# tumaer/lagrangebench

Measured on AMD Instinct MI355X. Metric: rollout particle-steps/sec, higher is better.
Workload: dtype f32 (GEMMs as fp16 hi/lo split products, fp32 accumulate)

## Files before the change

### include/lbhip.h

```cpp
#ifndef LBHIP_H
#define LBHIP_H

#include <stdint.h>

#ifdef __cplusplus
extern "C" {
#endif

#define LB_OK 0
#define LB_ERR_ARG (-1)
#define LB_ERR_HIP (-2)
#define LB_ERR_STATE (-3)
#define LB_ERR_DENSITY (-4)
#define LB_ERR_UNSUPPORTED (-5)

#define LB_FORCE_NONE 0
#define LB_FORCE_PIECEWISE 1
#define LB_FORCE_BUFFER 2

typedef struct lb_engine lb_engine;
typedef struct lb_gns lb_gns;

typedef struct lb_case_desc {
  int32_t dim;
// ... 38 lines not shown

int lb_set_force(lb_engine* eng, const double* force_dev);

int lb_load_window(lb_engine* eng, const double* traj_dev, int32_t T, int32_t t0, int32_t step);

int lb_read_window(lb_engine* eng, double* win_out_dev);


int lb_nl_allocate(lb_engine* eng, int32_t* cell_capacity_out, int32_t* e_cap_out,
                   int32_t* occupancy_out );

int lb_nl_set_capacity(lb_engine* eng, int32_t cell_capacity, int32_t e_cap);

int lb_nl_update(lb_engine* eng);

int lb_nl_read_flags(lb_engine* eng, int32_t* overflow_out_dev);

int lb_nl_read_idx(lb_engine* eng, int32_t* idx_out_dev, int32_t* n_edges_out_dev);


int lb_node_features(lb_engine* eng, double* vel_hist_out_dev, double* vel_mag_out_dev,
                     double* bound_out_dev, double* force_out_dev);

int lb_edge_features(lb_engine* eng, double* rel_disp_out_dev, double* rel_dist_out_dev);


int lb_gns_create(lb_engine* eng, const lb_gns_desc* desc, const float* weights_host,
                  int64_t n_floats, lb_gns** out);
void lb_gns_destroy(lb_gns* gns);

// ... 148 lines not shown
```

### lagrangebench_amd/_lib.py

```python
from __future__ import annotations

import ctypes as C
import os
from typing import Optional

_HERE = os.path.dirname(os.path.abspath(__file__))
LIB_PATH = os.path.join(_HERE, "csrc", "liblbhip.so")

LB_OK = 0
LB_FORCE_NONE, LB_FORCE_PIECEWISE, LB_FORCE_BUFFER = 0, 1, 2

D3 = C.c_double * 3


class CaseDesc(C.Structure):

    _fields_ = [
        ("dim", C.c_int32), ("n_particles", C.c_int32), ("batch", C.c_int32), ("isl", C.c_int32),
        ("periodic", C.c_int32), ("has_bound", C.c_int32), ("has_vel_mag", C.c_int32),
        ("force_kind", C.c_int32), ("force_axis", C.c_int32), ("geometry_f32", C.c_int32),
        ("box", D3), ("r_cutoff", C.c_double), ("capacity_multiplier", C.c_double),
        ("vel_mean", D3), ("vel_std", D3), ("acc_mean", D3), ("acc_std", D3),
        ("bound_lo", D3), ("bound_hi", D3),
        ("force_split", C.c_double), ("force_lo", D3), ("force_hi", D3),
# ... 45 lines not shown
_P = C.c_void_p
_SIGS = {
    "lb_strerror": (C.c_char_p, [C.c_int]),
    "lb_last_error": (C.c_char_p, []),
    "lb_version": (C.c_int, []),
    "lb_engine_create": (C.c_int, [C.POINTER(CaseDesc), _P, C.POINTER(_P)]),
    "lb_engine_destroy": (None, [_P]),
    "lb_set_particle_type": (C.c_int, [_P, _P]),
    "lb_set_force": (C.c_int, [_P, _P]),
    "lb_load_window": (C.c_int, [_P, _P, C.c_int32, C.c_int32, C.c_int32]),
    "lb_read_window": (C.c_int, [_P, _P]),
    "lb_nl_allocate": (C.c_int, [_P, C.POINTER(C.c_int32), C.POINTER(C.c_int32), C.POINTER(C.c_int32)]),
    "lb_nl_set_capacity": (C.c_int, [_P, C.c_int32, C.c_int32]),
    "lb_nl_update": (C.c_int, [_P]),
    "lb_nl_read_flags": (C.c_int, [_P, _P]),
    "lb_nl_read_idx": (C.c_int, [_P, _P, _P]),
    "lb_node_features": (C.c_int, [_P, _P, _P, _P, _P]),
    "lb_edge_features": (C.c_int, [_P, _P, _P]),
    "lb_gns_create": (C.c_int, [_P, C.POINTER(GnsDesc), _P, C.c_int64, C.POINTER(_P)]),
    "lb_gns_destroy": (None, [_P]),
    "lb_gns_forward": (C.c_int, [_P, _P, _P]),
    "lb_set_fused_aggregation": (C.c_int, [_P, C.c_int32]),
    "lb_gns_set_tap": (C.c_int, [_P, _P]),
    "lb_math_mode": (C.c_int, [_P, C.c_int32, C.POINTER(C.c_int32), C.POINTER(C.c_int32)]),
    "lb_math_fallbacks": (C.c_int32, [_P]),
    "lb_debug_inject_guard": (C.c_int, [_P, C.c_int32, C.c_int32]),
    "lb_integrate": (C.c_int, [_P, _P, _P, _P, C.c_int32]),
    "lb_case_integrate": (C.c_int, [_P, C.c_int32, _P, _P, C.c_int32, _P]),
    "lb_rollout": (C.c_int, [_P, _P, _P, C.c_int32, C.c_int32, _P, C.POINTER(C.c_int32)]),
    "lb_ekin": (C.c_int, [_P, _P, C.c_int32, C.c_int32, C.c_double, C.c_double, _P, C.c_int32]),
# ... 82 lines not shown
```

### lagrangebench_amd/csrc/lb_api.hip

```cpp
#include <cstddef>
#include <stdarg.h>
#include <stdio.h>
#include <stdlib.h>
#include <string.h>

#include <algorithm>
#include <cmath>

#include <initializer_list>
#include <tuple>

#include "lb_internal.h"
#include "lb_msplit.h"

thread_local std::string g_lb_err;

int lb_fail(int code, const char* fmt, ...) {
  char buf[1024];
  va_list ap;
  va_start(ap, fmt);
  vsnprintf(buf, sizeof(buf), fmt, ap);
  va_end(ap);
  g_lb_err = buf;
  return code;
// ... 221 lines not shown
  if (hipMemcpy(e->ctrl, &c0, sizeof(c0), hipMemcpyHostToDevice) != hipSuccess ||
      hipMemset(e->blocks_done, 0, sizeof(int32_t)) != hipSuccess ||
      hipMemset(e->ptype, 0, sizeof(int32_t) * BN) != hipSuccess ||
      hipMemset(e->nl_wg_sum, 0, sizeof(unsigned long long) * (BN / 8 + 2)) != hipSuccess ||
      hipMemset(e->row_ptr, 0, sizeof(int32_t) * (BN + 1)) != hipSuccess) {
    lb_engine_destroy(e);
    return lb_fail(LB_ERR_HIP, "engine init copies failed");
  }
  *out = e;
  return LB_OK;
}

extern "C" void lb_engine_destroy(lb_engine* e) {
  if (!e) return;
  lb_timers_collect(e);
  for (auto ev : e->epool) (void)hipEventDestroy(ev);
  void* bufs[] = {e->win, e->ptype, e->force, e->ctrl, e->cell_of, e->cell_count, e->cell_start,
                  e->cell_part, e->deg, e->nl_wg_sum, e->row_ptr, e->scan_part, e->cpos, e->tmp_send, e->tmp_feat, e->tmp_feat64,
                  e->senders, e->receivers, e->efeat, e->efeat64,
                  e->overflow, e->nedges_b, e->xnode, e->nlat, e->agg, e->psr, e->elat, e->msg,
                  e->acc, e->blocks_done};
  for (void* b : bufs)
    if (b) (void)hipFree(b);
  if (e->ctrl_host) (void)hipHostFree(e->ctrl_host);
  if (e->host_flag) (void)hipHostFree(e->host_flag);
  for (int i = 0; i < 4; ++i)
    if (e->step_ev[i]) (void)hipEventDestroy(e->step_ev[i]);
  if (e->gstream) (void)hipStreamDestroy(e->gstream);
  delete e;
}
// ... 114 lines not shown
    want = std::min<int32_t>(want, e->nl_dense ? LB_MAX_ROW_DENSE : LB_MAX_ROW);
    if (e->nl_dense) e->row_cap = std::max(e->row_cap, std::min<int32_t>((want + 63) / 64 * 64, LB_MAX_ROW_DENSE));
    if (want > e->maxd || !e->tmp_send) {
      LB_HIP(hipStreamSynchronize(e->stream));
      for (void* b : {(void*)e->tmp_send, (void*)e->tmp_feat, (void*)e->tmp_feat64})
        if (b) (void)hipFree(b);
      e->tmp_send = nullptr;
      e->tmp_feat = nullptr;
      e->tmp_feat64 = nullptr;
      e->maxd = want;
      LB_TRY(lb_alloc(&e->tmp_send, (size_t)e->BN * want));
      LB_TRY(lb_alloc(&e->tmp_feat, (size_t)e->BN * want * 4));
      LB_TRY(lb_alloc(&e->tmp_feat64, (size_t)e->BN * want * 4));
    }
  }
  if (cell_capacity_out) *cell_capacity_out = e->cell_capacity;
  if (e_cap_out) *e_cap_out = e->e_cap;
  if (occupancy_out) memcpy(occupancy_out, occ.data(), sizeof(int32_t) * e->g.B);
  return LB_OK;
}

extern "C" int lb_nl_set_capacity(lb_engine* e, int32_t cell_capacity, int32_t e_cap) {
  if (!e || e_cap < 1) return lb_fail(LB_ERR_ARG, "bad capacity");
  e->cell_capacity = cell_capacity;
  e->e_cap = e_cap;
  return lb_ensure_edges(e, (int64_t)e_cap * e->g.B);
}

extern "C" int lb_nl_update(lb_engine* e) {
  if (!e) return lb_fail(LB_ERR_ARG, "null engine");
// ... 672 lines not shown
      e->stream = s;
    }
  } restore{e, user_stream, &exec};
  if (use_graph) {
    if (!e->gstream) LB_HIP(hipStreamCreateWithFlags(&e->gstream, hipStreamNonBlocking));
    LB_HIP(hipEventRecord(e->step_ev[0], user_stream));
    LB_HIP(hipStreamWaitEvent(e->gstream, e->step_ev[0], 0));
    e->stream = e->gstream;
  }
  int n_realloc = 0, n_retry = 0;
  if (start_step > 0)
    LB_TRY(lbk_load_window_resume(e, traj_dev, T, pred_out_dev, n_steps, start_step));
  else
    LB_TRY(lbk_load_window(e, traj_dev, T, 0, 0));
  if (e->e_cap <= 0) LB_TRY(lb_nl_allocate(e, nullptr, nullptr, nullptr));
  int step = start_step;
  const int RA = 3;
  const int last = (stop_step >= 0 && stop_step < n_steps) ? stop_step : n_steps;
  while (step < last) {
    bool warm = false;
    for (int s = step; s < last; ++s) {
      if (s - step >= RA) {
        LB_HIP(hipEventSynchronize(e->step_ev[(s - RA) & 3]));
        if (*(volatile int32_t*)e->host_flag >= 0) break;
      }
      if (use_graph && warm && !exec) {
        hipGraph_t graph = nullptr;
        LB_HIP(hipStreamBeginCapture(e->stream, hipStreamCaptureModeThreadLocal));
        const int rc = lb_enqueue_step(e, forward, model, traj_dev, T, pred_out_dev, n_steps);
        const hipError_t ce = hipStreamEndCapture(e->stream, &graph);
// ... 36 lines not shown
      step = s_bad;
      if (++n_retry > 4) return lb_fail(LB_ERR_STATE, "single-launch paths keep timing out");
      continue;
    }
    LB_TRY(lb_check_density(e));
    if (e->ctrl_host->overflow_step < 0) break;
    step = e->ctrl_host->step;
    ++n_realloc;
    if (n_realloc > n_steps + 8) return lb_fail(LB_ERR_STATE, "neighbor list keeps overflowing");
    if (exec) {
      (void)hipGraphExecDestroy(exec);
      exec = nullptr;
    }
    LB_TRY(lb_nl_allocate(e, nullptr, nullptr, nullptr));
  }
  if (n_realloc_out) *n_realloc_out = n_realloc;
  return LB_OK;
}

extern "C" int lb_ekin(lb_engine* e, const double* rollout_dev, int32_t T, int32_t stride, double dt,
                       double dx, double* out_dev, int32_t n_out) {
  if (!e || !rollout_dev || !out_dev) return lb_fail(LB_ERR_ARG, "null argument");
  if (stride < 1 || T < 2) return lb_fail(LB_ERR_ARG, "need stride >= 1 and T >= 2");
  const int expect = (T - 1 + stride - 1) / stride;
  if (n_out != expect) return lb_fail(LB_ERR_ARG, "n_out must be ceil((T-1)/stride) = %d", expect);
  return lbk_ekin(e, rollout_dev, T, stride, n_out, dt, dx, out_dev);
}

extern "C" int lb_sinkhorn(lb_engine* e, const double* pred_dev, int32_t pred_T, const double* target_dev,
                           int32_t target_T, int32_t stride, double threshold, double* out_dev, int32_t n_out,
// ... 31 lines not shown
```

### lagrangebench_amd/csrc/lb_internal.h

```cpp
#pragma once
#include <cstdlib>
#include <hip/hip_ext.h>
#include <hip/hip_runtime.h>
#include <stdint.h>

#include <string>
#include <vector>

#include "../../include/lbhip.h"

#define LB_MAX_STENCIL_CAND 2048
#define LB_MAX_ROW 256
#define LB_MAX_ROW_DENSE 4096
#define LB_TILE 32
#define LB_D 128

typedef float f32x4 __attribute__((ext_vector_type(4)));
typedef float f32x16 __attribute__((ext_vector_type(16)));

struct lb_ctrl {
  int32_t step;
  int32_t overflow_step;
  int32_t n_edges_total;
  int32_t n_edges_unclamped;
  int32_t max_cell_occ;
  int32_t density_error;
  int32_t max_deg;
  int32_t row_overflow;
  int32_t math_flags;
  float ln_inv_d;
  float ln_pad;
  int32_t persist_error;
  int32_t nl_epoch;
  int32_t persist_step;
  int32_t math_step;
  int32_t acct_builds;
  int32_t acct_first;
  int64_t acct_sum;
};
__device__ __forceinline__ void lb_acct_edges(lb_ctrl* ctrl, int total) {
  if (ctrl->acct_builds == 0) ctrl->acct_first = total;
  ctrl->acct_builds += 1;
  ctrl->acct_sum += total;
}
#define LB_MATH_NO_STEP 0x7fffffff
#define LB_MATH_LARGE 1
#define LB_MATH_TINY 2
#define LB_MATH_NONFINITE 4

struct lb_geom {
  int32_t dim, N, B, isl, periodic, has_bound, has_vel_mag, force_kind, force_axis;
  int32_t use_cell_list;
  int32_t ncell[3];
// ... 71 lines not shown
  int32_t cell_capacity, e_cap;
  int64_t e_alloc;
  int32_t* cell_of;
  int32_t* cell_count;
  int32_t* cell_start;
  int32_t* cell_fill;
  bool cells_traj_ready = false;
  int32_t* cell_part;
  int32_t* deg;
  lb_feat_job feat_job{};
  bool feat_done = false;
  lb_integ_job integ_job{};
  bool integ_done = false;
  bool nl_one_off = false;
  unsigned long long* nl_wg_sum = nullptr;
  int32_t* row_ptr;
  int32_t* scan_part;
  double* cpos;
  int64_t cell_slots = 0;
  bool nl_dense = false;
  int32_t row_cap = 0;
  int32_t maxd;
  int32_t* tmp_send;
  float* tmp_feat;
  double* tmp_feat64;
  int32_t* senders;
  int32_t* receivers;
  float* efeat;
  double* efeat64;
  int32_t* overflow;
// ... 161 lines not shown
#define LB_LAUNCH_TIMED(e, kern, grid, block, ...)                                                        \
  do {                                                                                                    \
    if ((e)->ext_armed && !(e)->ext_used) {                                                               \
      hipExtLaunchKernelGGL(kern, grid, block, 0, (e)->stream, (e)->trecs.back().a, (e)->trecs.back().b, \
                            0, __VA_ARGS__);                                                              \
      (e)->ext_used = true;                                                                               \
    } else {                                                                                              \
      hipLaunchKernelGGL(kern, grid, block, 0, (e)->stream, __VA_ARGS__);                                 \
    }                                                                                                     \
  } while (0)

int lb_ensure_edges(lb_engine* e, int64_t need);
int lb_alloc_aggpart(lb_engine* e);

int lbk_nl_build(lb_engine* e, bool want_efeat64);
int lbk_nl_export(lb_engine* e, int32_t* idx_out, int32_t* n_edges_out);
int lbk_edge_features_export(lb_engine* e, double* rel_disp, double* rel_dist);

int lbk_load_window(lb_engine* e, const double* traj, int T, int t0, int step);
int lbk_load_window_resume(lb_engine* e, const double* traj, int T, const double* pred, int pred_T, int step);
int lbk_read_window(lb_engine* e, double* out);
int lbk_node_features(lb_engine* e, float* xnode, const float* embed, int emb, int ntypes,
                      double* vel_hist, double* vel_mag, double* bound, double* force);
int lbk_integrate(lb_engine* e, const float* acc, int acc_stride, const double* target,
                  const double* traj, int T, double* pred, int pred_T);
int lbk_ekin(lb_engine* e, const double* roll, int T, int stride, int n_out, double dt, double dx,
             double* out);
int lbk_case_integrate(lb_engine* e, int mode, const float* pred, const double* pos_seq, int T,
                       double* out);
int lbk_metrics(lb_engine* e, const double* pred, int pred_T, const double* target, int target_T,
// ... 74 lines not shown
```

### lagrangebench_amd/csrc/lb_neighbor.hip

```cpp
#include "lb_features.h"

#define SCAN_THREADS 256
#define SCAN_CHUNK (SCAN_THREADS * 8)
#define NL_SMALL_MAXC 1024

enum { NL_COUNT = 0, NL_FILL = 1, NL_ROWS = 2 };

__global__ void k_cell_count(lb_geom g, int64_t BN, const double* __restrict__ win,
                             lb_ctrl* __restrict__ ctrl, int32_t* __restrict__ cell_of,
                             int32_t* __restrict__ cell_count) {
  if (ctrl->overflow_step >= 0) return;
  int64_t gi = (int64_t)blockIdx.x * blockDim.x + threadIdx.x;
  if (gi == 0) {
    ctrl->max_cell_occ = 0;
    ctrl->max_deg = 0;
    ctrl->row_overflow = 0;
  }
  if (gi >= BN) return;
  const int step = ctrl->step;
  const int b = (int)(gi / g.N);
  int h = 0, mult = 1;
  for (int d = 0; d < g.dim; ++d) {
    double p = lb_pos(win, g, BN, step, g.isl - 1, d, gi);
    int c = __double2int_rz(lb_r(p / g.cell_size[d], g.f32));
// ... 85 lines not shown
  if (gi >= BN) return;
  const int step = ctrl->step;
  const int gc = cell_of[gi];
  const int slot = cell_start[gc] + atomicAdd(&cell_fill[gc], 1);
  cell_part[slot] = (int32_t)gi;
  for (int d = 0; d < g.dim; ++d) cpos[(int64_t)d * BN + slot] = lb_pos(win, g, BN, step, g.isl - 1, d, gi);
}

__global__ void k_cell_zero(lb_ctrl* __restrict__ ctrl, int32_t* __restrict__ cell_count, int n) {
  if (ctrl->overflow_step >= 0) return;
  const int i = blockIdx.x * blockDim.x + threadIdx.x;
  if (i == 0) {
    ctrl->max_cell_occ = 0;
    ctrl->max_deg = 0;
    ctrl->row_overflow = 0;
  }
  if (i < n) cell_count[i] = 0;
}
__global__ void __launch_bounds__(256) k_cell_bin(lb_geom g, int64_t BN, const double* __restrict__ win,
                                                  lb_ctrl* __restrict__ ctrl, int32_t* __restrict__ cell_of,
                                                  int32_t* __restrict__ cell_count, int32_t* __restrict__ cell_part,
                                                  double* __restrict__ cpos, int32_t cap, int64_t cstride) {
  if (ctrl->overflow_step >= 0) return;
  const int64_t gi = (int64_t)blockIdx.x * blockDim.x + threadIdx.x;
  const int step = ctrl->step;
  int occ = 0;
  if (gi < BN) {
    const int b = (int)(gi / g.N);
    int h = 0, mult = 1;
    double p[3] = {0, 0, 0};
// ... 269 lines not shown
  const int32_t* cell_start;
  const int32_t* cell_part;
  const double* cpos;
  const int32_t* cell_cnt;
  int32_t cell_cap;
  int64_t cstride;
  int32_t* deg;
  const int32_t* row_ptr;
  lb_edge_out out;
  int64_t e_alloc;
  int32_t maxd;
  int32_t row_cap;
  lb_feat_job feat;
  const double* win;
  int32_t nb_search;
};
#define NL_FEAT_ROWS 8
__device__ __forceinline__ int lb_cell_begin(const lb_nl_args& a, int gc) { return a.cell_cap ? gc * a.cell_cap : a.cell_start[gc]; }
__device__ __forceinline__ int lb_cell_size(const lb_nl_args& a, int gc, int begin) {
  return a.cell_cap ? min(a.cell_cnt[gc], a.cell_cap) : a.cell_start[gc + 1] - begin;
}


__device__ __forceinline__ void lb_load_pos(double* p, const double* src, int64_t stride, int64_t i, int dim) {
#pragma unroll
  for (int d = 0; d < 3; ++d) p[d] = d < dim ? src[d * stride + i] : 0.0;
}

template <bool F32, typename PS>
__device__ __forceinline__ bool lb_pair_in_cutoff(const lb_geom& g, PS ps, const double* pr, int dim) {
  double dd = lb_disp1(ps(0), pr[0], g.box[0], g.half_box[0], g.periodic, F32);
// ... 80 lines not shown
  return s_cstart[lo] + (j - s_coff[lo]);
}

__device__ __forceinline__ bool lb_feature_rows(const lb_geom& g, int64_t BN, const lb_ctrl* ctrl, const lb_nl_args& a,
                                                int waves) {
  if (a.nb_search <= 0 || (int)blockIdx.x < a.nb_search) return false;
  const int64_t first = ((int64_t)(blockIdx.x - a.nb_search) * waves + (threadIdx.x >> 6)) * NL_FEAT_ROWS;
  const int cnt = (int)min((int64_t)NL_FEAT_ROWS, BN - first);
  if (cnt > 0)
    lb_node_features_wave_multi(g, BN, a.win, ctrl->step, a.feat, [&](int p) -> int64_t { return first + p; }, cnt);
  return true;
}

template <int MODE>
__device__ __forceinline__ int lb_cap_row(lb_ctrl* ctrl, const lb_nl_args& a, int count, int lane, int row_cap, bool can_grow) {
  if (count > row_cap) {
    if (lane == 0) {
      if (MODE == NL_ROWS && can_grow)
        atomicExch(&ctrl->row_overflow, 1);
      else
        atomicExch(&ctrl->density_error, 2);
    }
    count = row_cap;
  }
  if (MODE == NL_ROWS && count > a.maxd) {
    if (lane == 0) atomicExch(&ctrl->row_overflow, 1);
    count = a.maxd;
  }
  return count;
}

__device__ __forceinline__ int lb_rank_in_row(int my, int count) {
  int rank = 0;
  for (int u = 0; u < count; ++u) rank += (__builtin_amdgcn_readlane(my, u) < my) ? 1 : 0;
  return rank;
}

template <int MODE, int NL_THREADS, int MAXC>
__global__ void __launch_bounds__(NL_THREADS)
    k_nl(lb_geom g, int64_t BN, lb_ctrl* __restrict__ ctrl, lb_nl_args a) {
// ... 144 lines not shown
                                          g.dim);
  }
}

#define NLC_WAVES 4
#define NLC_LIST 448
#define NLC_BATCH 128
#define NLC_S 4
template <int MODE, bool F32, int DIM>
__global__ void __launch_bounds__(64 * NLC_WAVES, 5)
    k_nlc(lb_geom g, int64_t BN, lb_ctrl* __restrict__ ctrl, lb_nl_args a) {
  __shared__ int s_cstart_[NLC_WAVES][28], s_coff_[NLC_WAVES][29];
  __shared__ int s_src_[NLC_WAVES][NLC_LIST], s_id_[NLC_WAVES][NLC_LIST];
  __shared__ unsigned short s_kr_[NLC_WAVES][NLC_LIST];
  if (ctrl->overflow_step >= 0) return;
  if (MODE == NL_ROWS && lb_feature_rows(g, BN, ctrl, a, NLC_WAVES)) return;
  const int wave = threadIdx.x >> 6, lane = threadIdx.x & 63;
  const int gc = __builtin_amdgcn_readfirstlane((int)blockIdx.x * NLC_WAVES + wave);
  if (gc >= g.B * g.ncells) return;
  const int own_start = lb_cell_begin(a, gc);
  const int own_cnt = lb_cell_size(a, gc, own_start);
  if (own_cnt <= 0) return;
  int* const s_cstart = s_cstart_[wave];
  int* const s_coff = s_coff_[wave];
  int* const s_src = s_src_[wave];
  int* const s_id = s_id_[wave];
  unsigned short* const s_kr = s_kr_[wave];
  lb_stencil_table(g, a, gc, lane, DIM, s_cstart, s_coff);
  __builtin_amdgcn_fence(__ATOMIC_SEQ_CST, "wavefront");
  const int M = __builtin_amdgcn_readfirstlane(s_coff[g.nstencil]);
  const bool single = M <= 64 * NLC_S;
  const unsigned long long lt_mask = (lane == 0) ? 0ull : (~0ull >> (64 - lane));
  int cj[NLC_S], cid[NLC_S];
  auto load_chunk = [&](int c0) {
#pragma unroll
    for (int s = 0; s < NLC_S; ++s) {
      if (c0 + 64 * s >= M) continue;
      cj[s] = lb_stencil_slot(s_cstart, s_coff, g.nstencil, min(c0 + 64 * s + lane, M - 1));
      cid[s] = a.cell_part[cj[s]];
    }
  };
  const int cap = (MODE == NL_ROWS) ? min(a.maxd, LB_MAX_ROW) : LB_MAX_ROW;
  int list_len = 0, kfirst = 0;
  auto flush = [&]() {
    __builtin_amdgcn_fence(__ATOMIC_SEQ_CST, "wavefront");
    for (int t0 = 0; t0 < list_len; t0 += 64) {
      const int t = t0 + lane;
      const bool act = t < list_len;
      const int tc = act ? t : 0;
      const int src = s_src[tc], my = s_id[tc], kr = s_kr[tc];
      const int rslot = own_start + kfirst + (kr >> 8), rank = kr & 0xff;
      const int gr = a.cell_part[rslot];
      double pr[DIM], sp[DIM];
#pragma unroll
      for (int d = 0; d < DIM; ++d) {
        pr[d] = a.cpos[(int64_t)d * a.cstride + rslot];
        sp[d] = a.cpos[(int64_t)d * a.cstride + src];
      }
      if (!act) continue;
      const int64_t base = (MODE == NL_ROWS) ? (int64_t)gr * a.maxd : (int64_t)a.row_ptr[gr];
      const int64_t slot = base + rank;
      if (MODE == NL_ROWS || slot < a.e_alloc)
        lb_write_edge<F32, MODE == NL_ROWS>(g, a.out, slot, my, gr, pr, [&](int d) { return sp[d]; }, DIM);
    }
    __builtin_amdgcn_fence(__ATOMIC_SEQ_CST, "wavefront");
  };
#pragma unroll
  for (int s = 0; s < NLC_S; ++s) cj[s] = cid[s] = 0;
  if (single) load_chunk(0);
  float q[NLC_S][DIM];
#pragma unroll
  for (int s = 0; s < NLC_S; ++s)
    _Pragma("unroll") for (int d = 0; d < DIM; ++d) q[s][d] = 0.f;
  bool filt = false;
  const float lo2 = (float)(g.rc2 * (1.0 - 1e-4)), hi2 = (float)(g.rc2 * (1.0 + 1e-4));
// ... 85 lines not shown
    if (MODE == NL_COUNT) continue;
    count = lb_cap_row<MODE>(ctrl, a, count, lane, LB_MAX_ROW, true);
    __builtin_amdgcn_fence(__ATOMIC_SEQ_CST, "wavefront");
    if (count <= 64) {
      const int rank = lb_rank_in_row(s_id[list_len + min(lane, max(count - 1, 0))], count);
      if (lane < count) s_kr[list_len + lane] = (unsigned short)((kb << 8) | rank);
    } else {
      for (int t = lane; t < count; t += 64) {
        const int my = s_id[list_len + t];
        int rank = 0;
        for (int u = 0; u < count; ++u) rank += (s_id[list_len + u] < my) ? 1 : 0;
        s_kr[list_len + t] = (unsigned short)((kb << 8) | rank);
      }
    }
    list_len += count;
  }
}

__device__ __forceinline__ void lb_copy_row(int64_t gnode, int d, int64_t base, int32_t maxd, const int32_t* __restrict__ tsend,
                                            const float* __restrict__ tfeat, const double* __restrict__ tfeat64,
                                            int32_t* __restrict__ senders, int32_t* __restrict__ receivers,
                                            float* __restrict__ efeat, double* __restrict__ efeat64, int64_t e_alloc) {
  for (int k = threadIdx.x & 15; k < d; k += 16) {
    const int64_t src = gnode * maxd + k, dst = base + k;
    if (dst >= e_alloc) break;
    senders[dst] = tsend[src];
    receivers[dst] = (int32_t)gnode;
    f32x4* ef = reinterpret_cast<f32x4*>(efeat + dst * 8);
    ef[0] = reinterpret_cast<const f32x4*>(tfeat)[src];
    ef[1] = f32x4{0.f, 0.f, 0.f, 0.f};
// ... 654 lines not shown
  a.host_flag = e->host_flag_dev;
  if (e->feat_job.xnode && !want_efeat64) {
    a.feat = e->feat_job;
    e->feat_done = true;
  }
  return a;
}

#define LB_NLS_MAX_LDS (150 * 1024)
template <bool F32, int DIM>
static void lb_launch_one_traj(lb_engine* e, bool mid, int nb, int threads, size_t lds, const lb_nls_args& a) {
  if (mid)
    lb_launch_lds<k_nl_mid<F32, DIM>>(LB_NLS_MAX_LDS, dim3(nb), dim3(threads), lds, e->stream, e->g, e->ctrl, a);
  else
    lb_launch_lds<k_nl_small<F32, DIM>>(LB_NLS_MAX_LDS, dim3(nb), dim3(threads), lds, e->stream, e->g, e->ctrl, a);
}

int lbk_nl_build(lb_engine* e, bool want_efeat64) {
  const lb_geom& g = e->g;
  const int64_t BN = e->BN;
  const int ncell_tot = g.B * g.ncells;
  hipStream_t s = e->stream;
  const int frozen = e->e_cap > 0;

  const bool small_ok = lb_fused_launches();
  const bool small_rows = small_ok && BN <= LB_SMALL_N;
  const bool small_cells = small_rows && ncell_tot <= LB_SMALL_N;
  static_assert(NLS_CAND >= LB_MAX_ROW, "k_nl_small's row buffer holds a full row");
  const bool one_traj = small_ok && frozen && g.B == 1 && !e->nl_dense && !e->nl_one_off && e->nl_wg_sum &&
                        g.ncell[0] < 2048 && g.ncell[1] < 2048 && g.ncell[2] < 1024;
// ... 18 lines not shown
    lb_toc(e);
    LB_HIP(hipGetLastError());
    return LB_OK;
  }
  lb_tic(e, LB_T_CELLS);
  const bool mid_cells = small_ok && frozen && g.B == 1 && BN <= LB_CELLS1_N && ncell_tot <= LB_CELLS1_NCELL;
  const bool traj_cells = small_ok && frozen && !small_cells && g.B > 1 && g.use_cell_list && g.N <= 6144 &&
                          g.ncells <= LB_CELLS1_NCELL;
  const int64_t strided_slots = (int64_t)ncell_tot * e->cell_capacity;
#ifdef LB_NO_STRIDED
  const bool strided = false;
#else
  const bool strided = small_ok && frozen && g.use_cell_list && e->cell_capacity > 0 && lb_nl_kernel_kind(e) != 1 &&
                       strided_slots < ((int64_t)1 << 30);
#endif
  if (strided) {
    if (strided_slots > e->cell_slots) {
      LB_HIP(hipStreamSynchronize(s));
      if (e->cell_part) (void)hipFree(e->cell_part);
      if (e->cpos) (void)hipFree(e->cpos);
      e->cell_part = nullptr;
      e->cpos = nullptr;
      e->cell_slots = strided_slots + strided_slots / 4;
      LB_HIP(hipMalloc((void**)&e->cell_part, sizeof(int32_t) * (size_t)e->cell_slots));
      LB_HIP(hipMalloc((void**)&e->cpos, sizeof(double) * (size_t)g.dim * (size_t)e->cell_slots));
    }
    e->cells_traj_ready = false;
    hipLaunchKernelGGL(k_cell_zero, dim3((ncell_tot + 255) / 256), dim3(256), 0, s, e->ctrl, e->cell_count, ncell_tot);
    hipLaunchKernelGGL(k_cell_bin, dim3((unsigned)((BN + 255) / 256)), dim3(256), 0, s, g, BN, e->win, e->ctrl, e->cell_of,
                       e->cell_count, e->cell_part, e->cpos, e->cell_capacity, strided_slots);
  } else if (small_cells) {
// ... 32 lines not shown
  const int small = (frozen && g.use_cell_list && cand_cap <= NL_SMALL_MAXC)
                        ? (int)std::max<int64_t>(128, (cand_cap + 127) / 128 * 128) : 0;
  const bool rows = frozen && e->maxd > 0 && e->tmp_send && (!want_efeat64 || e->tmp_feat64);
  lb_nl_args a{};
  a.cell_of = e->cell_of;
  a.cell_start = e->cell_start;
  a.cell_part = e->cell_part;
  a.cpos = e->cpos;
  a.cell_cnt = e->cell_count;
  a.cell_cap = strided ? e->cell_capacity : 0;
  a.cstride = strided ? strided_slots : BN;
  a.deg = e->deg;
  a.row_ptr = e->row_ptr;
  a.e_alloc = e->e_alloc;
  a.maxd = e->maxd;
  if (rows) {
    a.out = {e->tmp_send, nullptr, e->tmp_feat, want_efeat64 ? e->tmp_feat64 : nullptr};
    lb_launch_nl<NL_ROWS>(e, small, a);
  } else {
    lb_launch_nl<NL_COUNT>(e, small, a);
  }
  if (rows && small_ok && BN <= LB_CSCAN_N && g.B <= 64) {
    hipLaunchKernelGGL(k_nl_compact_scan, dim3((int)((BN + 15) / 16)), dim3(256), 0, s, g, BN, e->ctrl, e->deg, e->row_ptr,
                       e->maxd, e->tmp_send, e->tmp_feat, want_efeat64 ? e->tmp_feat64 : (const double*)nullptr,
                       e->senders, e->receivers, e->efeat, want_efeat64 ? e->efeat64 : (double*)nullptr, e->e_alloc,
                       e->overflow, e->nedges_b, e->cell_capacity, e->e_cap, e->host_flag_dev);
    lb_toc(e);
    LB_HIP(hipGetLastError());
    return LB_OK;
  }
  if (small_rows) {
// ... 111 lines not shown
```

### lagrangebench_amd/engine.py

```python
from __future__ import annotations

import ctypes as C
from typing import Dict, List, Optional, Sequence, Tuple

import numpy as np
import torch

from . import _lib
from ._lib import CaseDesc, EgnnDesc, GnsDesc, LbHipError, PainnDesc, SegnnDesc, check, ptr


def _d3(v, fill=0.0):
    a = [fill, fill, fill]
    for i, x in enumerate(list(v)[:3]):
        a[i] = float(x)
    return _lib.D3(*a)


def _dev(t: torch.Tensor, dtype, device) -> torch.Tensor:
    return t.to(device=device, dtype=dtype).contiguous()


class ForceSpec:

# ... 139 lines not shown
        cc, ec = C.c_int32(), C.c_int32()
        occ = (C.c_int32 * self.B)()
        check(self.lib.lb_nl_allocate(self._h, C.byref(cc), C.byref(ec), occ), "lb_nl_allocate")
        self.cell_capacity, self.e_cap = cc.value, ec.value
        self.version += 1
        return cc.value, ec.value, list(occ)

    def nl_set_capacity(self, cell_capacity: int, e_cap: int) -> None:
        check(self.lib.lb_nl_set_capacity(self._h, int(cell_capacity), int(e_cap)), "lb_nl_set_capacity")
        self.cell_capacity, self.e_cap = int(cell_capacity), int(e_cap)

    def nl_update(self) -> None:
        check(self.lib.lb_nl_update(self._h), "lb_nl_update")
        self.version += 1

    def nl_flags(self) -> torch.Tensor:
        out = torch.empty((self.B,), dtype=torch.int32, device=self.device)
        check(self.lib.lb_nl_read_flags(self._h, ptr(out)), "lb_nl_read_flags")
        return out

    def nl_idx(self) -> Tuple[torch.Tensor, torch.Tensor]:
        idx = torch.empty((self.B, 2, self.e_cap), dtype=torch.int32, device=self.device)
        ne = torch.empty((self.B,), dtype=torch.int32, device=self.device)
        check(self.lib.lb_nl_read_idx(self._h, ptr(idx), ptr(ne)), "lb_nl_read_idx")
        return idx, ne

    def stats(self) -> Dict[str, int]:
        n, ec, cc = C.c_int64(), C.c_int32(), C.c_int32()
        check(self.lib.lb_stats(self._h, C.byref(n), C.byref(ec), C.byref(cc)), "lb_stats")
        return {"n_edges_total": n.value, "e_cap": ec.value, "cell_capacity": cc.value}
# ... 425 lines not shown
```

Baseline: 21.34 million.

## Add Verlet skin neighbor list with displacement-triggered candidate rebuilds

Introduces a Verlet-style skin: a candidate list is built on a coarser grid with cutoff rc+skin, and it is rebuilt only when the max particle displacement since the last build exceeds half the skin. Each step a check kernel computes displacements and cell ids, and a filter kernel prunes candidates to true neighbors within rc. This is meant to cut the cost of the full cell-list search each step. In exchange it adds memory, extra kernels, and a heuristic that turns the skin off when rebuilds are too frequent. It is limited to 3D, f64 geometry and the strided cell path.

```diff
diff --git a/include/lbhip.h b/include/lbhip.h
--- a/include/lbhip.h
+++ b/include/lbhip.h
@@ -76,6 +76,11 @@
 
 int lb_nl_update(lb_engine* eng);
 
+int lb_nl_skin(lb_engine* eng, int32_t mode, double* skin_out, int32_t* builds_out);
+
+int lb_nl_skin_plan(const lb_case_desc* desc, int32_t max_deg, int32_t cell_capacity, double* skin_out,
+                    int32_t* cand_cap_out, int32_t* skin_cell_cap_out);
+
 int lb_nl_read_flags(lb_engine* eng, int32_t* overflow_out_dev);
 
 int lb_nl_read_idx(lb_engine* eng, int32_t* idx_out_dev, int32_t* n_edges_out_dev);
diff --git a/lagrangebench_amd/_lib.py b/lagrangebench_amd/_lib.py
--- a/lagrangebench_amd/_lib.py
+++ b/lagrangebench_amd/_lib.py
@@ -83,6 +83,8 @@
     "lb_nl_set_capacity": (C.c_int, [_P, C.c_int32, C.c_int32]),
     "lb_nl_update": (C.c_int, [_P]),
     "lb_nl_read_flags": (C.c_int, [_P, _P]),
+    "lb_nl_skin": (C.c_int, [_P, C.c_int32, C.POINTER(C.c_double), C.POINTER(C.c_int32)]),
+    "lb_nl_skin_plan": (C.c_int, [_P, C.c_int32, C.c_int32, C.POINTER(C.c_double), C.POINTER(C.c_int32), C.POINTER(C.c_int32)]),
     "lb_nl_read_idx": (C.c_int, [_P, _P, _P]),
     "lb_node_features": (C.c_int, [_P, _P, _P, _P, _P]),
     "lb_edge_features": (C.c_int, [_P, _P, _P]),
diff --git a/lagrangebench_amd/csrc/lb_api.hip b/lagrangebench_amd/csrc/lb_api.hip
--- a/lagrangebench_amd/csrc/lb_api.hip
+++ b/lagrangebench_amd/csrc/lb_api.hip
@@ -259,6 +259,7 @@
 extern "C" void lb_engine_destroy(lb_engine* e) {
   if (!e) return;
   lb_timers_collect(e);
+  lb_skin_free(e);
   for (auto ev : e->epool) (void)hipEventDestroy(ev);
   void* bufs[] = {e->win, e->ptype, e->force, e->ctrl, e->cell_of, e->cell_count, e->cell_start,
                   e->cell_part, e->deg, e->nl_wg_sum, e->row_ptr, e->scan_part, e->cpos, e->tmp_send, e->tmp_feat, e->tmp_feat64,
@@ -403,6 +404,7 @@
       LB_TRY(lb_alloc(&e->tmp_feat64, (size_t)e->BN * want * 4));
     }
   }
+  LB_TRY(lb_skin_setup(e, h->max_deg, h->skin_cmax, h->skin_occ));
   if (cell_capacity_out) *cell_capacity_out = e->cell_capacity;
   if (e_cap_out) *e_cap_out = e->e_cap;
   if (occupancy_out) memcpy(occupancy_out, occ.data(), sizeof(int32_t) * e->g.B);
@@ -1105,6 +1107,7 @@
   else
     LB_TRY(lbk_load_window(e, traj_dev, T, 0, 0));
   if (e->e_cap <= 0) LB_TRY(lb_nl_allocate(e, nullptr, nullptr, nullptr));
+  if (e->skin > 0) LB_HIP(hipMemsetAsync(&e->ctrl->skin_roll_builds, 0, sizeof(int32_t), e->stream));
   int step = start_step;
   const int RA = 3;
   const int last = (stop_step >= 0 && stop_step < n_steps) ? stop_step : n_steps;
@@ -1171,6 +1174,10 @@
     }
     LB_TRY(lb_nl_allocate(e, nullptr, nullptr, nullptr));
   }
+  if (e->skin > 0 && last - start_step >= 8 && 3 * (e->ctrl_host->skin_roll_builds - 1) > last - start_step) {
+    e->skin_off = true;
+    e->skin = 0.0;
+  }
   if (n_realloc_out) *n_realloc_out = n_realloc;
   return LB_OK;
 }
diff --git a/lagrangebench_amd/csrc/lb_internal.h b/lagrangebench_amd/csrc/lb_internal.h
--- a/lagrangebench_amd/csrc/lb_internal.h
+++ b/lagrangebench_amd/csrc/lb_internal.h
@@ -37,6 +37,12 @@
   int32_t acct_builds;
   int32_t acct_first;
   int64_t acct_sum;
+  int32_t skin_stale;
+  int32_t skin_cmax;
+  int32_t skin_occ;
+  int32_t skin_builds;
+  int32_t skin_roll_builds;
+  unsigned long long skin_disp2;
 };
 __device__ __forceinline__ void lb_acct_edges(lb_ctrl* ctrl, int total) {
   if (ctrl->acct_builds == 0) ctrl->acct_first = total;
@@ -138,6 +144,21 @@
   bool integ_done = false;
   bool nl_one_off = false;
   unsigned long long* nl_wg_sum = nullptr;
+  lb_geom gs{};
+  double skin = 0.0;
+  double skin_thr2 = 0.0;
+  bool skin_off = false;
+  bool skin_disabled = false;
+  int32_t skin_cap = 0;
+  int32_t ccap = 0;
+  int64_t skin_cells_alloc = 0, skin_cand_alloc = 0;
+  int32_t* skin_count = nullptr;
+  int32_t* skin_part = nullptr;
+  double* skin_pos = nullptr;
+  double* refpos = nullptr;
+  int32_t* cand = nullptr;
+  int32_t* ccnt = nullptr;
+  int32_t* cellc = nullptr;
   int32_t* row_ptr;
   int32_t* scan_part;
   double* cpos;
@@ -329,6 +350,8 @@
 int lb_alloc_aggpart(lb_engine* e);
 
 int lbk_nl_build(lb_engine* e, bool want_efeat64);
+int lb_skin_setup(lb_engine* e, int32_t max_deg, int32_t cmax_seen, int32_t occ_seen);
+void lb_skin_free(lb_engine* e);
 int lbk_nl_export(lb_engine* e, int32_t* idx_out, int32_t* n_edges_out);
 int lbk_edge_features_export(lb_engine* e, double* rel_disp, double* rel_dist);
 
diff --git a/lagrangebench_amd/csrc/lb_neighbor.hip b/lagrangebench_amd/csrc/lb_neighbor.hip
--- a/lagrangebench_amd/csrc/lb_neighbor.hip
+++ b/lagrangebench_amd/csrc/lb_neighbor.hip
@@ -4,7 +4,7 @@
 #define SCAN_CHUNK (SCAN_THREADS * 8)
 #define NL_SMALL_MAXC 1024
 
-enum { NL_COUNT = 0, NL_FILL = 1, NL_ROWS = 2 };
+enum { NL_COUNT = 0, NL_FILL = 1, NL_ROWS = 2, NL_CAND = 3 };
 
 __global__ void k_cell_count(lb_geom g, int64_t BN, const double* __restrict__ win,
                              lb_ctrl* __restrict__ ctrl, int32_t* __restrict__ cell_of,
@@ -123,6 +123,7 @@
     ctrl->max_cell_occ = 0;
     ctrl->max_deg = 0;
     ctrl->row_overflow = 0;
+    ctrl->skin_disp2 = 0ull;
   }
   if (i < n) cell_count[i] = 0;
 }
@@ -422,7 +423,15 @@
   lb_feat_job feat;
   const double* win;
   int32_t nb_search;
+  const int32_t* cand;
+  const int32_t* ccnt;
+  int32_t ccap;
+  const int32_t* cellc;
+  double skin_thr2;
 };
+__device__ __forceinline__ bool lb_skin_due(const lb_ctrl* ctrl, double thr2) {
+  return ctrl->skin_stale || !(__longlong_as_double((long long)ctrl->skin_disp2) <= thr2);
+}
 #define NL_FEAT_ROWS 8
 __device__ __forceinline__ int lb_cell_begin(const lb_nl_args& a, int gc) { return a.cell_cap ? gc * a.cell_cap : a.cell_start[gc]; }
 __device__ __forceinline__ int lb_cell_size(const lb_nl_args& a, int gc, int begin) {
@@ -533,16 +542,17 @@
 
 template <int MODE>
 __device__ __forceinline__ int lb_cap_row(lb_ctrl* ctrl, const lb_nl_args& a, int count, int lane, int row_cap, bool can_grow) {
+  if (MODE == NL_CAND && count > min(a.maxd, row_cap) && lane == 0) atomicMax(&ctrl->skin_cmax, count);
   if (count > row_cap) {
     if (lane == 0) {
-      if (MODE == NL_ROWS && can_grow)
+      if (MODE >= NL_ROWS && can_grow)
         atomicExch(&ctrl->row_overflow, 1);
       else
         atomicExch(&ctrl->density_error, 2);
     }
     count = row_cap;
   }
-  if (MODE == NL_ROWS && count > a.maxd) {
+  if (MODE >= NL_ROWS && count > a.maxd) {
     if (lane == 0) atomicExch(&ctrl->row_overflow, 1);
     count = a.maxd;
   }
@@ -717,6 +727,7 @@
   __shared__ int s_src_[NLC_WAVES][NLC_LIST], s_id_[NLC_WAVES][NLC_LIST];
   __shared__ unsigned short s_kr_[NLC_WAVES][NLC_LIST];
   if (ctrl->overflow_step >= 0) return;
+  if (MODE == NL_CAND && !lb_skin_due(ctrl, a.skin_thr2)) return;
   if (MODE == NL_ROWS && lb_feature_rows(g, BN, ctrl, a, NLC_WAVES)) return;
   const int wave = threadIdx.x >> 6, lane = threadIdx.x & 63;
   const int gc = __builtin_amdgcn_readfirstlane((int)blockIdx.x * NLC_WAVES + wave);
@@ -743,7 +754,7 @@
       cid[s] = a.cell_part[cj[s]];
     }
   };
-  const int cap = (MODE == NL_ROWS) ? min(a.maxd, LB_MAX_ROW) : LB_MAX_ROW;
+  const int cap = (MODE >= NL_ROWS) ? min(a.maxd, LB_MAX_ROW) : LB_MAX_ROW;
   int list_len = 0, kfirst = 0;
   auto flush = [&]() {
     __builtin_amdgcn_fence(__ATOMIC_SEQ_CST, "wavefront");
@@ -754,6 +765,10 @@
       const int src = s_src[tc], my = s_id[tc], kr = s_kr[tc];
       const int rslot = own_start + kfirst + (kr >> 8), rank = kr & 0xff;
       const int gr = a.cell_part[rslot];
+      if (MODE == NL_CAND) {
+        if (act) a.out.senders[(int64_t)gr * a.maxd + rank] = my;
+        continue;
+      }
       double pr[DIM], sp[DIM];
 #pragma unroll
       for (int d = 0; d < DIM; ++d) {
@@ -761,7 +776,7 @@
         sp[d] = a.cpos[(int64_t)d * a.cstride + src];
       }
       if (!act) continue;
-      const int64_t base = (MODE == NL_ROWS) ? (int64_t)gr * a.maxd : (int64_t)a.row_ptr[gr];
+      const int64_t base = (MODE >= NL_ROWS) ? (int64_t)gr * a.maxd : (int64_t)a.row_ptr[gr];
       const int64_t slot = base + rank;
       if (MODE == NL_ROWS || slot < a.e_alloc)
         lb_write_edge<F32, MODE == NL_ROWS>(g, a.out, slot, my, gr, pr, [&](int d) { return sp[d]; }, DIM);
@@ -877,6 +892,133 @@
       }
     }
     list_len += count;
+  }
+}
+
+
+__device__ __forceinline__ int lb_rc_cell(const lb_geom& g, double p, int d) {
+  const int c = __double2int_rz(lb_r(p / g.cell_size[d], g.f32));
+  return c < 0 ? 0 : (c >= g.ncell[d] ? g.ncell[d] - 1 : c);
+}
+
+__global__ void __launch_bounds__(256)
+    k_skin_check(lb_geom g, int64_t BN, const double* __restrict__ win, lb_ctrl* __restrict__ ctrl,
+                 int32_t* __restrict__ cell_of, int32_t* __restrict__ cell_count, int32_t* __restrict__ cellc,
+                 const double* __restrict__ refpos, int32_t* __restrict__ skin_count, int nskin) {
+  if (ctrl->overflow_step >= 0) return;
+  const int64_t gi = (int64_t)blockIdx.x * blockDim.x + threadIdx.x;
+  if (gi < nskin) skin_count[gi] = 0;
+  const int step = ctrl->step;
+  double d2 = 0.0;
+  if (gi < BN) {
+    const int b = (int)(gi / g.N);
+    int h = 0, mult = 1, packed = 0;
+    for (int d = 0; d < g.dim; ++d) {
+      const double p = lb_pos(win, g, BN, step, g.isl - 1, d, gi);
+      const int c = lb_rc_cell(g, p, d);
+      h += c * mult;
+      mult *= g.ncell[d];
+      packed |= c << (10 * d);
+      const double dd = lb_disp1(p, refpos[(int64_t)d * BN + gi], g.box[d], g.half_box[d], g.periodic);
+      d2 += dd * dd;
+    }
+    if (!(d2 <= 1e300)) d2 = INFINITY;
+    const int gc = b * g.ncells + h;
+    cell_of[gi] = gc;
+    cellc[gi] = packed;
+    atomicAdd(&cell_count[gc], 1);
+  }
+  for (int o = 32; o > 0; o >>= 1) d2 = fmax(d2, __shfl_xor(d2, o));
+  if ((threadIdx.x & 63) == 0 && d2 > 0.0) atomicMax(&ctrl->skin_disp2, (unsigned long long)__double_as_longlong(d2));
+}
+
+__global__ void __launch_bounds__(256)
+    k_skin_bin(lb_geom gs, int64_t BN, const double* __restrict__ win, lb_ctrl* __restrict__ ctrl,
+               const int32_t* __restrict__ cell_count, int ncell_tot, int32_t* __restrict__ skin_count,
+               int32_t* __restrict__ skin_part, double* __restrict__ skin_pos, double* __restrict__ refpos, int32_t cap,
+               int64_t cstride, double thr2) {
+  if (ctrl->overflow_step >= 0) return;
+  const int64_t gi = (int64_t)blockIdx.x * blockDim.x + threadIdx.x;
+  int occ = gi < ncell_tot ? cell_count[gi] : 0;
+  for (int o = 32; o > 0; o >>= 1) occ = max(occ, __shfl_xor(occ, o));
+  if ((threadIdx.x & 63) == 0 && occ > 0) atomicMax(&ctrl->max_cell_occ, occ);
+  if (!lb_skin_due(ctrl, thr2)) return;
+  if (gi == 0) {
+    ctrl->skin_builds += 1;
+    ctrl->skin_roll_builds += 1;
+  }
+  if (gi >= BN) return;
+  const int step = ctrl->step;
+  const int b = (int)(gi / gs.N);
+  int h = 0, mult = 1;
+  double p[3] = {0, 0, 0};
+  for (int d = 0; d < gs.dim; ++d) {
+    p[d] = lb_pos(win, gs, BN, step, gs.isl - 1, d, gi);
+    refpos[(int64_t)d * BN + gi] = p[d];
+    const double w = gs.periodic ? lb_mod(p[d], gs.box[d]) : p[d];
+    int c = __double2int_rz(w / gs.cell_size[d]);
+    c = c < 0 ? 0 : (c >= gs.ncell[d] ? gs.ncell[d] - 1 : c);
+    h += c * mult;
+    mult *= gs.ncell[d];
+  }
+  const int gc = b * gs.ncells + h;
+  const int slot = atomicAdd(&skin_count[gc], 1);
+  if (slot < cap) {
+    const int64_t idx = (int64_t)gc * cap + slot;
+    skin_part[idx] = (int32_t)gi;
+    for (int d = 0; d < gs.dim; ++d) skin_pos[(int64_t)d * cstride + idx] = p[d];
+  } else {
+    atomicExch(&ctrl->row_overflow, 1);
+    atomicMax(&ctrl->skin_occ, slot + 1);
+  }
+}
+
+__device__ __forceinline__ bool lb_rc_adjacent(const lb_geom& g, int ca, int cb, int dim) {
+  bool ok = true;
+  for (int d = 0; d < dim; ++d) {
+    const int df = abs(((ca >> (10 * d)) & 1023) - ((cb >> (10 * d)) & 1023));
+    ok = ok && (df <= 1 || df == g.ncell[d] - 1);
+  }
+  return ok;
+}
+
+#define SKF_WAVES 4
+template <int DIM>
+__global__ void __launch_bounds__(64 * SKF_WAVES)
+    k_skin_filter(lb_geom g, int64_t BN, lb_ctrl* __restrict__ ctrl, lb_nl_args a) {
+  if (ctrl->overflow_step >= 0) return;
+  if (blockIdx.x == 0 && threadIdx.x == 0 && ctrl->skin_stale) ctrl->skin_stale = 0;
+  if (lb_feature_rows(g, BN, ctrl, a, SKF_WAVES)) return;
+  const int lane = threadIdx.x & 63, l = lane & 31;
+  const int64_t gr = ((int64_t)blockIdx.x * SKF_WAVES + (threadIdx.x >> 6)) * 2 + (lane >> 5);
+  if (gr >= BN) return;
+  const int step = ctrl->step;
+  double pr[DIM];
+#pragma unroll
+  for (int d = 0; d < DIM; ++d) pr[d] = lb_pos(a.win, g, BN, step, g.isl - 1, d, gr);
+  const int ccr = a.cellc[gr];
+  const int n = min(a.ccnt[gr], a.ccap);
+  const int cap = min(a.maxd, LB_MAX_ROW);
+  const int32_t* row = a.cand + gr * a.ccap;
+  int count = 0;
+  for (int c0 = 0; c0 < n; c0 += 32) {
+    const int j = c0 + l;
+    const int sj = row[min(j, a.ccap - 1)];
+    const bool act = j < n;
+    const int s = act ? sj : (int)gr;
+    double sp[DIM];
+#pragma unroll
+    for (int d = 0; d < DIM; ++d) sp[d] = lb_pos(a.win, g, BN, step, g.isl - 1, d, s);
+    const auto ps = [&](int d) { return sp[d]; };
+    const bool hit = act && lb_rc_adjacent(g, a.cellc[s], ccr, DIM) && lb_pair_in_cutoff<false>(g, ps, pr, DIM);
+    const unsigned m = (unsigned)(__ballot(hit) >> (lane & 32));
+    const int p = count + __popc(m & ((1u << l) - 1u));
+    if (hit && p < cap) lb_write_edge<false, true>(g, a.out, gr * a.maxd + p, s, (int)gr, pr, ps, DIM);
+    count += __popc(m);
+  }
+  if (l == 0) {
+    a.deg[gr] = count;
+    if (count > cap) atomicExch(&ctrl->row_overflow, 1);
   }
 }
 
@@ -1561,6 +1703,146 @@
     lb_launch_lds<k_nl_mid<F32, DIM>>(LB_NLS_MAX_LDS, dim3(nb), dim3(threads), lds, e->stream, e->g, e->ctrl, a);
   else
     lb_launch_lds<k_nl_small<F32, DIM>>(LB_NLS_MAX_LDS, dim3(nb), dim3(threads), lds, e->stream, e->g, e->ctrl, a);
+}
+
+#define LB_SKIN_FRAC 0.25
+#define LB_SKIN_BUDGET ((int64_t)512 << 20)
+struct lb_skin_plan_t {
+  double skin = 0.0;
+  int32_t ncell[3] = {1, 1, 1};
+  int32_t ccap = 0, cell_cap = 0;
+  int64_t bytes = 0;
+};
+static lb_skin_plan_t lb_skin_plan(int dim, int f32, int use_cell_list, const int32_t* ncell, const double* box, double rc,
+                                   int64_t B, int64_t N, int32_t max_deg, int32_t cell_capacity, int32_t cmax_seen,
+                                   int32_t occ_seen) {
+  lb_skin_plan_t p;
+#ifndef LB_NO_SKIN
+  if (dim != 3 || f32 || !use_cell_list || !(rc > 0) || max_deg < 1 || cell_capacity < 1) return p;
+  const double skin = LB_SKIN_FRAC * rc, R = rc + skin;
+  double ratio = 1.0;
+  int64_t ncells = 1;
+  for (int d = 0; d < dim; ++d) {
+    if (ncell[d] > 1024) return p;
+    const double n = std::floor(box[d] / (R * (1.0 + 1e-6)));
+    if (!(n >= 3.0) || n > 1024.0) return p;
+    p.ncell[d] = (int32_t)n;
+    ratio *= (box[d] / n) / (box[d] / ncell[d]);
+    ncells *= p.ncell[d];
+  }
+  const double grow = std::pow(R / rc, dim);
+  int64_t ccap = (int64_t)std::ceil(max_deg * grow * 1.25);
+  ccap = std::max<int64_t>(ccap, (int64_t)std::ceil(cmax_seen * 1.25));
+  ccap = std::max<int64_t>(16, (ccap + 7) / 8 * 8);
+  if (ccap > LB_MAX_ROW) return p;
+  int64_t cc = (int64_t)std::ceil(cell_capacity * ratio * 1.25) + 2;
+  cc = std::max<int64_t>(cc, (int64_t)std::ceil(occ_seen * 1.25));
+  p.bytes = B * N * ccap * 4 + B * ncells * cc * (4 + 8 * dim) + B * ncells * 4 + B * N * (8 * dim + 8);
+  if (p.bytes > LB_SKIN_BUDGET || (int64_t)B * ncells * cc >= ((int64_t)1 << 30)) return p;
+  p.skin = skin;
+  p.ccap = (int32_t)ccap;
+  p.cell_cap = (int32_t)cc;
+#endif
+  return p;
+}
+
+extern "C" int lb_nl_skin_plan(const lb_case_desc* d, int32_t max_deg, int32_t cell_capacity, double* skin_out,
+                               int32_t* cand_cap_out, int32_t* skin_cell_cap_out) {
+  if (!d || !skin_out) return lb_fail(LB_ERR_ARG, "null argument");
+  if (d->dim != 2 && d->dim != 3) return lb_fail(LB_ERR_ARG, "dim must be 2 or 3 (got %d)", d->dim);
+  int32_t ncell[3] = {1, 1, 1};
+  double box[3] = {1, 1, 1};
+  int use = 1;
+  for (int k = 0; k < d->dim; ++k) {
+    const float b32 = (float)d->box[k];
+    if (!((float)d->r_cutoff < b32 / 3.0f)) use = 0;
+    ncell[k] = (int32_t)floorf(b32 / (float)d->r_cutoff);
+    box[k] = d->box[k];
+  }
+  const lb_skin_plan_t p = lb_skin_plan(d->dim, d->geometry_f32 != 0, use, ncell, box, d->r_cutoff, d->batch, d->n_particles,
+                                        max_deg, cell_capacity, 0, 0);
+  *skin_out = p.skin;
+  if (cand_cap_out) *cand_cap_out = p.ccap;
+  if (skin_cell_cap_out) *skin_cell_cap_out = p.cell_cap;
+  return LB_OK;
+}
+
+extern "C" int lb_nl_skin(lb_engine* e, int32_t mode, double* skin_out, int32_t* builds_out) {
+  if (!e) return lb_fail(LB_ERR_ARG, "null engine");
+  if (mode == 0) {
+    e->skin_disabled = true;
+    e->skin = 0.0;
+  } else if (mode == 1) {
+    e->skin_disabled = false;
+  }
+  if (skin_out) *skin_out = e->skin;
+  if (builds_out) {
+    LB_HIP(hipMemcpyAsync(&e->ctrl_host->skin_builds, &e->ctrl->skin_builds, sizeof(int32_t), hipMemcpyDeviceToHost, e->stream));
+    LB_HIP(hipStreamSynchronize(e->stream));
+    *builds_out = e->ctrl_host->skin_builds;
+  }
+  return LB_OK;
+}
+
+void lb_skin_free(lb_engine* e) {
+  for (void* b : {(void*)e->skin_count, (void*)e->skin_part, (void*)e->skin_pos, (void*)e->refpos, (void*)e->cand,
+                  (void*)e->ccnt, (void*)e->cellc})
+    if (b) (void)hipFree(b);
+  e->skin_count = e->skin_part = e->cand = e->ccnt = e->cellc = nullptr;
+  e->skin_pos = e->refpos = nullptr;
+  e->skin_cells_alloc = e->skin_cand_alloc = 0;
+}
+
+int lb_skin_setup(lb_engine* e, int32_t max_deg, int32_t cmax_seen, int32_t occ_seen) {
+  const lb_geom& g = e->g;
+  if (cmax_seen > LB_MAX_ROW) e->skin_off = true;
+  lb_skin_plan_t p;
+  if (!e->skin_off && !e->skin_disabled && !e->nl_dense)
+    p = lb_skin_plan(g.dim, g.f32, g.use_cell_list, g.ncell, g.box, g.rc, g.B, g.N, max_deg, e->cell_capacity, cmax_seen,
+                     occ_seen);
+  e->skin = p.skin;
+  if (p.skin <= 0) return LB_OK;
+  p.ccap = std::max(p.ccap, std::min(e->ccap, LB_MAX_ROW));
+  p.cell_cap = std::max(p.cell_cap, e->skin_cap);
+  lb_geom& gs = e->gs;
+  gs = g;
+  gs.rc = g.rc + p.skin;
+  gs.rc2 = gs.rc * gs.rc;
+  gs.ncells = 1;
+  for (int d = 0; d < 3; ++d) {
+    gs.ncell[d] = d < g.dim ? p.ncell[d] : 1;
+    gs.cell_size[d] = d < g.dim ? g.box[d] / p.ncell[d] : 1.0;
+    gs.ncells *= gs.ncell[d];
+  }
+  const double thr = 0.5 * p.skin - 1e-6 * gs.rc;
+  e->skin_thr2 = thr * thr;
+  e->skin_cap = p.cell_cap;
+  e->ccap = p.ccap;
+  const int64_t cells = (int64_t)g.B * gs.ncells * p.cell_cap, cand = e->BN * p.ccap;
+  if (cells > e->skin_cells_alloc || cand > e->skin_cand_alloc || !e->refpos) {
+    LB_HIP(hipStreamSynchronize(e->stream));
+    lb_skin_free(e);
+    LB_TRY(lb_alloc(&e->skin_count, (size_t)g.B * gs.ncells));
+    LB_TRY(lb_alloc(&e->skin_part, (size_t)cells));
+    LB_TRY(lb_alloc(&e->skin_pos, (size_t)cells * g.dim));
+    LB_TRY(lb_alloc(&e->refpos, (size_t)e->BN * g.dim));
+    LB_TRY(lb_alloc(&e->cand, (size_t)cand));
+    LB_TRY(lb_alloc(&e->ccnt, (size_t)e->BN));
+    LB_TRY(lb_alloc(&e->cellc, (size_t)e->BN));
+    LB_HIP(hipMemsetAsync(e->ccnt, 0, sizeof(int32_t) * (size_t)e->BN, e->stream));
+    e->skin_cells_alloc = cells;
+    e->skin_cand_alloc = cand;
+  }
+  lb_ctrl* h = e->ctrl_host;
+  h->skin_stale = 1;
+  h->skin_cmax = 0;
+  h->skin_occ = 0;
+  LB_HIP(hipMemcpyAsync(&e->ctrl->skin_stale, &h->skin_stale, offsetof(lb_ctrl, skin_builds) - offsetof(lb_ctrl, skin_stale),
+                        hipMemcpyHostToDevice, e->stream));
+  h->skin_disp2 = 0ull;
+  LB_HIP(hipMemcpyAsync(&e->ctrl->skin_disp2, &h->skin_disp2, sizeof(h->skin_disp2), hipMemcpyHostToDevice, e->stream));
+  LB_HIP(hipStreamSynchronize(e->stream));
+  return LB_OK;
 }
 
 int lbk_nl_build(lb_engine* e, bool want_efeat64) {
@@ -1609,7 +1891,18 @@
   const bool strided = small_ok && frozen && g.use_cell_list && e->cell_capacity > 0 && lb_nl_kernel_kind(e) != 1 &&
                        strided_slots < ((int64_t)1 << 30);
 #endif
-  if (strided) {
+  const bool skin = strided && e->skin > 0 && e->ccap > 0 && e->maxd > 0 && e->tmp_send && (!want_efeat64 || e->tmp_feat64) &&
+                    lb_nl_kernel_kind(e) == 2 && !g.f32 && g.dim == 3;
+  if (skin) {
+    const int nskin = g.B * e->gs.ncells;
+    e->cells_traj_ready = false;
+    hipLaunchKernelGGL(k_cell_zero, dim3((ncell_tot + 255) / 256), dim3(256), 0, s, e->ctrl, e->cell_count, ncell_tot);
+    hipLaunchKernelGGL(k_skin_check, dim3((unsigned)((std::max<int64_t>(BN, nskin) + 255) / 256)), dim3(256), 0, s, g, BN, e->win,
+                       e->ctrl, e->cell_of, e->cell_count, e->cellc, (const double*)e->refpos, e->skin_count, nskin);
+    hipLaunchKernelGGL(k_skin_bin, dim3((unsigned)((std::max<int64_t>(BN, ncell_tot) + 255) / 256)), dim3(256), 0, s, e->gs, BN,
+                       e->win, e->ctrl, (const int32_t*)e->cell_count, ncell_tot, e->skin_count, e->skin_part, e->skin_pos,
+                       e->refpos, e->skin_cap, (int64_t)nskin * e->skin_cap, e->skin_thr2);
+  } else if (strided) {
     if (strided_slots > e->cell_slots) {
       LB_HIP(hipStreamSynchronize(s));
       if (e->cell_part) (void)hipFree(e->cell_part);
@@ -1672,7 +1965,36 @@
   a.row_ptr = e->row_ptr;
   a.e_alloc = e->e_alloc;
   a.maxd = e->maxd;
-  if (rows) {
+  if (skin) {
+    const int nskin = e->g.B * e->gs.ncells;
+    lb_nl_args c{};
+    c.cell_part = e->skin_part;
+    c.cpos = e->skin_pos;
+    c.cell_cnt = e->skin_count;
+    c.cell_cap = e->skin_cap;
+    c.cstride = (int64_t)nskin * e->skin_cap;
+    c.deg = e->ccnt;
+    c.out = {e->cand, nullptr, nullptr, nullptr};
+    c.maxd = e->ccap;
+    c.skin_thr2 = e->skin_thr2;
+    hipLaunchKernelGGL((k_nlc<NL_CAND, false, 3>), dim3((nskin + NLC_WAVES - 1) / NLC_WAVES), dim3(64 * NLC_WAVES), 0, s, e->gs, BN,
+                       e->ctrl, c);
+    a.out = {e->tmp_send, nullptr, e->tmp_feat, want_efeat64 ? e->tmp_feat64 : nullptr};
+    a.win = e->win;
+    a.cand = e->cand;
+    a.ccnt = e->ccnt;
+    a.ccap = e->ccap;
+    a.cellc = e->cellc;
+    const int64_t nb_f = (BN + 2 * SKF_WAVES - 1) / (2 * SKF_WAVES);
+    int64_t nb = nb_f;
+    if (e->feat_job.xnode && !want_efeat64) {
+      e->feat_done = true;
+      a.feat = e->feat_job;
+      a.nb_search = (int)nb_f;
+      nb += (BN + SKF_WAVES * NL_FEAT_ROWS - 1) / (SKF_WAVES * NL_FEAT_ROWS);
+    }
+    hipLaunchKernelGGL(k_skin_filter<3>, dim3((unsigned)nb), dim3(64 * SKF_WAVES), 0, s, g, BN, e->ctrl, a);
+  } else if (rows) {
     a.out = {e->tmp_send, nullptr, e->tmp_feat, want_efeat64 ? e->tmp_feat64 : nullptr};
     lb_launch_nl<NL_ROWS>(e, small, a);
   } else {
diff --git a/lagrangebench_amd/engine.py b/lagrangebench_amd/engine.py
--- a/lagrangebench_amd/engine.py
+++ b/lagrangebench_amd/engine.py
@@ -177,6 +177,11 @@
         check(self.lib.lb_nl_update(self._h), "lb_nl_update")
         self.version += 1
 
+    def nl_skin(self, mode: int = -1) -> Tuple[float, int]:
+        sk, nb = C.c_double(), C.c_int32()
+        check(self.lib.lb_nl_skin(self._h, int(mode), C.byref(sk), C.byref(nb)), "lb_nl_skin")
+        return sk.value, nb.value
+
     def nl_flags(self) -> torch.Tensor:
         out = torch.empty((self.B,), dtype=torch.int32, device=self.device)
         check(self.lib.lb_nl_read_flags(self._h, ptr(out)), "lb_nl_read_flags")
```

Result: no change. 21.34 million, median of 5 (+0.0%).
